# rafaelcgon/2D-GP

Hardware: AMD Instinct MI355X
Metric: posterior grid points/sec (fit+predict), N_train=4096, div-free 2D kernel (higher is better)
Workload: dtype f64 (variance GEMM as exact int8 Ozaki-II); 1 GPU; df kernel, N_train=4096, 256x256 grid per GPU, fit+predict (mean+variance); n_train=4096, grid_per_gpu=256x256, points_total=65536, parallelism=grid-sharded x1, factor local, kstar_ahead=False

## Files before the change

### 2d-gp_amd/csrc/ozaki.hpp

```cpp
#pragma once
#include <climits>
#include <type_traits>
#include "common.hpp"
#include "assemble.hpp"

namespace gp2d {

constexpr int OZ_MAXMOD = 20;
#ifdef GP2D_OZ_P
#define GP2D_OZ_PW GP2D_OZ_P
#define GP2D_OZ_PB GP2D_OZ_P
#endif
#ifndef GP2D_OZ_PW
#define GP2D_OZ_PW 49
#endif
#ifndef GP2D_OZ_PB
#define GP2D_OZ_PB 45
#endif
constexpr int OZ_PW = GP2D_OZ_PW;
constexpr int OZ_PB = GP2D_OZ_PB;
static_assert(OZ_PW <= 50 && OZ_PB <= 50, "ozaki: the one-part residues need |x| < 2^50");
constexpr int OZ_PW_MAX = 60;
constexpr int OZ_PB_MAX = 50;
constexpr int OZ_SPLIT = 26;
constexpr int OZ_HBITS = 33;

struct OzakiConsts {
  int nmod;
  int pw;
  int pb;
  int m[OZ_MAXMOD];
  double c26[OZ_MAXMOD];
  double md[OZ_MAXMOD];
  double inv_m[OZ_MAXMOD];
  double h[OZ_MAXMOD];
  double t[OZ_MAXMOD];
  double M;
  int sB;
  double vlimit;
};

constexpr double OZ_MAGIC52 = 6755399441055744.0;
__device__ __forceinline__ uint32_t residue_low_m(double x, double xm, double m, double inv_m) {
  return (uint32_t)__double_as_longlong(fma(-m, rint(x * inv_m), xm));
}
__device__ __forceinline__ uint32_t pack2_lo(uint32_t a, uint32_t b) { return __builtin_amdgcn_perm(b, a, 0x0c0c0400u); }
__device__ __forceinline__ uint32_t pack22(uint32_t a, uint32_t b) { return __builtin_amdgcn_perm(b, a, 0x05040100u); }

__host__ __device__ __forceinline__ int64_t slab_offset(int64_t row, int64_t k, int64_t K) {
  return (((row >> 8) * (K >> 6) + (k >> 6)) << 14) + ((row & 255) << 6) + (k & 63);
}

__device__ __forceinline__ double block_reduce(double v, double* red, bool is_max) {
  const int tid = threadIdx.x;
  red[tid] = v;
  __syncthreads();
  for (int s = 128; s > 0; s >>= 1) {
    if (tid < s) red[tid] = is_max ? fmax(red[tid], red[tid + s]) : red[tid] + red[tid + s];
    __syncthreads();
  }
  const double r = red[0];
  __syncthreads();
  return r;
}

struct WRows {
  int64_t ldw;
  __device__ __forceinline__ int64_t off(int64_t i) const {
    if (ldw) return i * ldw;
    const int64_t rb = i >> 7;
    return ((rb * (rb + 1)) << 13) + (i & 127) * ((rb + 1) << 7);
  }
  __device__ __forceinline__ int64_t len(int64_t i, int64_t n) const { return ldw ? n : ((i >> 7) + 1) << 7; }
};

__global__ __launch_bounds__(256) void ozaki_w_scale_kernel(const double* __restrict__ W, int64_t n, WRows wr, int pw,
                                                            double* __restrict__ rowscale, double* __restrict__ l1,
                                                            double M, int sB, int final_scale) {
  __shared__ double red[256];
  const int64_t i = blockIdx.x;
  const int tid = threadIdx.x;
  const double* w = W + wr.off(i);
  double mx = 0.0;
  for (int64_t k = tid; k <= i; k += 256) mx = fmax(mx, fabs(w[k]));
  mx = block_reduce(mx, red, true);
  const int e = (mx > 0.0) ? ilogb(mx) : 0;
  const int si = pw - 1 - e;
  double sum = 0.0;
  if (l1 != nullptr) {
    for (int64_t k = tid; k <= i; k += 256) sum += fabs(rint(ldexp(w[k], si)));
    sum = block_reduce(sum, red, false);
  }
  if (tid == 0) {
    rowscale[i] = final_scale ? ldexp(M, -si - sB) : (double)si;
    if (l1 != nullptr) l1[i] = sum;
  }
}

__global__ __launch_bounds__(256) void ozaki_rowscale_final_kernel(double* __restrict__ rowscale, int64_t n, double M,
                                                                   int sB) {
  const int64_t i = (int64_t)blockIdx.x * 256 + threadIdx.x;
  if (i < n) rowscale[i] = ldexp(M, -(int)rowscale[i] - sB);
}

__device__ __forceinline__ int ozaki_row_exp(double rowscale_i, const OzakiConsts& oc) {
  return ilogb(oc.M) - ilogb(rowscale_i) - oc.sB;
}

__device__ __forceinline__ void w_residues4(const double (&x)[4], const OzakiConsts& oc, int l, uint32_t (&r)[4]) {
  const double m = oc.md[l], im = oc.inv_m[l];
  if (oc.pw <= 50) {
#pragma unroll
    for (int u = 0; u < 4; ++u) r[u] = residue_low_m(x[u], x[u] + OZ_MAGIC52, m, im);
  } else {
    const double c = oc.c26[l];
#pragma unroll
    for (int u = 0; u < 4; ++u) {
      const double xh = rint(ldexp(x[u], -OZ_SPLIT));
      const double xl = x[u] - ldexp(xh, OZ_SPLIT);
      const double rh = fma(-m, rint(xh * im), xh), rl = fma(-m, rint(xl * im), xl);
      const double t = fma(rh, c, rl);
      r[u] = residue_low_m(t, t + OZ_MAGIC52, m, im);
    }
  }
}
__device__ __forceinline__ uint32_t pack4_lo(const uint32_t (&r)[4]) {
  return pack22(pack2_lo(r[0], r[1]), pack2_lo(r[2], r[3]));
}
__device__ __forceinline__ uint32_t centred_sum(uint32_t a, uint32_t b, int m) {
  int s = (int)a + (int)b;
  const int half = m >> 1;
  s -= (s > half) ? m : 0;
  s += (s < -half) ? m : 0;
  return (uint32_t)s;
}

__global__ __launch_bounds__(256) void ozaki_w_res_kernel(const double* __restrict__ W, int64_t n, WRows wr,
                                                          OzakiConsts oc, int8_t* __restrict__ wres,
                                                          const double* __restrict__ rowscale, int64_t s_npad) {
  const int64_t bi = blockIdx.y, ks = blockIdx.x;
  if (ks * 64 >= (bi + 1) * 256) return;
  const int64_t hs = s_npad / 64;
  const bool fold = hs > 0 && bi * 256 >= s_npad;
  if (fold && ks >= hs) return;
  const bool right = fold && (ks + hs) * 64 < (bi + 1) * 256;
  const int lane = threadIdx.x & 63, wv = threadIdx.x >> 6;
  const int64_t k0 = ks * 64 + 4 * (lane & 15);
  const int64_t plane = n * n;
  auto scaled4 = [&](int64_t i, int64_t kc, int si, double (&x)[4]) {
    const double* w = W + wr.off(i) + kc;
    d2 p0 = {0.0, 0.0}, p1 = {0.0, 0.0};
    if (kc < wr.len(i, n)) {
      p0 = *reinterpret_cast<const d2*>(w);
      p1 = *reinterpret_cast<const d2*>(w + 2);
    }
    const double v[4] = {p0.x, p0.y, p1.x, p1.y};
#pragma unroll
    for (int u = 0; u < 4; ++u) x[u] = (kc + u <= i) ? rint(ldexp(v[u], si)) : 0.0;
  };
#pragma unroll 1
  for (int it = 0; it < 16; ++it) {
    const int64_t i = bi * 256 + wv * 64 + it * 4 + (lane >> 4);
    const int si = ozaki_row_exp(rowscale[i], oc);
    double x[4];
    scaled4(i, k0, si, x);
    int8_t* dst = wres + slab_offset(i, k0, n);
    if (!fold) {
      for (int l = 0; l < oc.nmod; ++l) {
        uint32_t r[4];
        w_residues4(x, oc, l, r);
        *reinterpret_cast<uint32_t*>(dst + (int64_t)l * plane) = pack4_lo(r);
      }
    } else {
      double xr[4] = {0.0, 0.0, 0.0, 0.0};
      if (right) scaled4(i, s_npad + k0, si, xr);
      int8_t* dst_r = wres + slab_offset(i, s_npad + k0, n);
      int8_t* dst_s = wres + slab_offset(i - s_npad, s_npad + k0, n);
      for (int l = 0; l < oc.nmod; ++l) {
        uint32_t r[4], q[4] = {0u, 0u, 0u, 0u};
        w_residues4(x, oc, l, r);
        *reinterpret_cast<uint32_t*>(dst + (int64_t)l * plane) = pack4_lo(r);
        if (right) {
          w_residues4(xr, oc, l, q);
          *reinterpret_cast<uint32_t*>(dst_r + (int64_t)l * plane) = pack4_lo(q);
        }
#pragma unroll
        for (int u = 0; u < 4; ++u) q[u] = centred_sum(r[u], q[u], oc.m[l]);
        *reinterpret_cast<uint32_t*>(dst_s + (int64_t)l * plane) = pack4_lo(q);
      }
    }
  }
}

#ifndef GP2D_KS_OCC
#define GP2D_KS_OCC 5
#endif
#ifndef GP2D_KS_PPL
#define GP2D_KS_PPL 2
#endif
constexpr int OZ_KS_T = 64;
constexpr int OZ_KS_P = 64;
constexpr int OZ_KS_PPL = GP2D_KS_PPL;
static_assert(OZ_KS_PPL == 2 || OZ_KS_PPL == 4, "2 or 4 training points per lane");

template <int PPL> struct packed_bytes;
template <> struct packed_bytes<2> { typedef uint16_t type; };
template <> struct packed_bytes<4> { typedef uint32_t type; };

enum { KS_PLAIN = 0, KS_DIFF_X = 1, KS_DIFF_R = 2 };
template <bool OFF32, int FORM>
__global__ __launch_bounds__(256, GP2D_KS_OCC) void ozaki_kstar_kernel(
    const double* __restrict__ xtr, int64_t ntr, int64_t npad, const double* __restrict__ xg, int64_t cv,
    int64_t cp, VecParams vp, const double* __restrict__ alpha, OzakiConsts oc, int8_t* __restrict__ bres,
    double* __restrict__ pm, uint8_t* __restrict__ flags) {
  constexpr int PPL = OZ_KS_PPL, LG = 64 / PPL, RPW = 64 / LG, RPI = 4 * RPW;
  typedef typename packed_bytes<PPL>::type pk_t;
  const int lane = threadIdx.x & 63, wv = threadIdx.x >> 6;
  const int kg = lane % LG, r = lane / LG;
  const int64_t t0 = (int64_t)blockIdx.x * OZ_KS_T + PPL * kg;
  const int64_t n = 2 * npad, ncols = 2 * cp;
  double a1[PPL], a2[PPL], x0[PPL], x1[PPL], x2[PPL];
  bool tv[PPL];
#pragma unroll
  for (int u = 0; u < PPL; ++u) {
    const int64_t t = t0 + u;
    tv[u] = t < ntr;
    x0[u] = x1[u] = x2[u] = 0.0;
    if (tv[u]) vec_point(vp, xtr, t, x0[u], x1[u], x2[u]);
    a1[u] = (alpha != nullptr && t < npad) ? alpha[t] : 0.0;
    a2[u] = (alpha != nullptr && t < npad) ? alpha[npad + t] : 0.0;
  }
  const double scale = ldexp(1.0, oc.sB);
  bool nz = false;
#pragma unroll 1
  for (int q = 0; q < OZ_KS_P / RPI; ++q) {
    const int64_t p = (int64_t)blockIdx.y * OZ_KS_P + RPI * q + RPW * wv + r;
    const bool pv = p < cv;
    double g0 = 0.0, g1 = 0.0, g2 = 0.0;
    if (pv) vec_point(vp, xg, p, g0, g1, g2);
    double k11[PPL], k12[PPL], k22[PPL];
    double mu = 0.0, mv = 0.0;
#pragma unroll
    for (int u = 0; u < PPL; ++u) {
      if (pv && tv[u]) {
        vec_block_st(vp, x0[u] - g0, x1[u] - g1, x2[u] - g2, k11[u], k12[u], k22[u]);
      } else {
        k11[u] = k12[u] = k22[u] = 0.0;
      }
      mu += a1[u] * k11[u] + a2[u] * k12[u];
      mv += a1[u] * k12[u] + a2[u] * k22[u];
    }
    if (pm != nullptr) {
#pragma unroll
      for (int o = LG / 2; o > 0; o >>= 1) {
        mu += __shfl_xor(mu, o);
        mv += __shfl_xor(mv, o);
      }
      if (kg == 0 && p < cp) {
        pm[(int64_t)blockIdx.x * ncols + p] = mu;
        pm[(int64_t)blockIdx.x * ncols + cp + p] = mv;
      }
    }
    if (p >= cp || t0 >= npad) continue;
    double xi[3][PPL], xm[3][PPL];
#pragma unroll
    for (int u = 0; u < PPL; ++u) {
      xi[0][u] = rint(k11[u] * scale);
      xi[1][u] = rint(k12[u] * scale);
      xi[2][u] = rint(k22[u] * scale);
      if constexpr (FORM == KS_DIFF_X) {
        xi[0][u] -= xi[1][u];
        xi[2][u] -= xi[1][u];
      }
      if constexpr (FORM == KS_DIFF_R) nz = nz || xi[1][u] != 0.0 || xi[0][u] != xi[1][u] || xi[2][u] != xi[1][u];
      else nz = nz || xi[0][u] != 0.0 || xi[1][u] != 0.0 || xi[2][u] != 0.0;
#pragma unroll
      for (int e = 0; e < 3; ++e) xm[e][u] = xi[e][u] + OZ_MAGIC52;
    }
    const int64_t o_uu = slab_offset(p, t0, n), o_uv = slab_offset(p, npad + t0, n),
                  o_vv = slab_offset(cp + p, npad + t0, n);
    const int64_t pstride = ncols * n;
    for (int l = 0; l < oc.nmod; ++l) {
      const double m = oc.md[l], im = oc.inv_m[l];
      pk_t pk[3];
      uint32_t r[3][PPL];
#pragma unroll
      for (int e = 0; e < 3; ++e)
#pragma unroll
        for (int u = 0; u < PPL; ++u) r[e][u] = residue_low_m(xi[e][u], xm[e][u], m, im);
      if constexpr (FORM == KS_DIFF_R) {
#pragma unroll
        for (int u = 0; u < PPL; ++u) {
          r[0][u] = centred_sum(r[0][u], 0u - r[1][u], oc.m[l]);
          r[2][u] = centred_sum(r[2][u], 0u - r[1][u], oc.m[l]);
        }
      }
#pragma unroll
      for (int e = 0; e < 3; ++e) {
        if constexpr (PPL == 2) pk[e] = (pk_t)pack2_lo(r[e][0], r[e][1]);
        else pk[e] = (pk_t)pack22(pack2_lo(r[e][0], r[e][1]), pack2_lo(r[e][2], r[e][3]));
      }
      int8_t* plane = bres + (int64_t)l * pstride;
      if constexpr (OFF32) {
        const __amdgpu_buffer_rsrc_t rs = __builtin_amdgcn_make_buffer_rsrc(plane, (short)0, (int)pstride, 0x00020000);
        if constexpr (PPL == 2) {
          __builtin_amdgcn_raw_buffer_store_b16(pk[0], rs, (int)o_uu, 0, 0);
          __builtin_amdgcn_raw_buffer_store_b16(pk[1], rs, (int)o_uv, 0, 0);
          __builtin_amdgcn_raw_buffer_store_b16(pk[2], rs, (int)o_vv, 0, 0);
        } else {
          __builtin_amdgcn_raw_buffer_store_b32(pk[0], rs, (int)o_uu, 0, 0);
          __builtin_amdgcn_raw_buffer_store_b32(pk[1], rs, (int)o_uv, 0, 0);
          __builtin_amdgcn_raw_buffer_store_b32(pk[2], rs, (int)o_vv, 0, 0);
        }
      } else {
        *reinterpret_cast<pk_t*>(plane + o_uu) = pk[0];
        *reinterpret_cast<pk_t*>(plane + o_uv) = pk[1];
        *reinterpret_cast<pk_t*>(plane + o_vv) = pk[2];
      }
    }
  }
  if (flags != nullptr) {
    const int any = __syncthreads_or(nz ? 1 : 0);
    if (threadIdx.x == 0) flags[(int64_t)blockIdx.y * gridDim.x + blockIdx.x] = any ? 1 : 0;
  }
}

__global__ __launch_bounds__(64) void ozaki_slab_list_kernel(const uint8_t* __restrict__ flags, int ntb, int nbj,
                                                             int kslabs, int* __restrict__ list,
                                                             int* __restrict__ cnt) {
  const int bj = blockIdx.x, lane = threadIdx.x;
  const int g = bj % (nbj / 2);
  const uint8_t* f = flags + (int64_t)(4 * g) * ntb;
  int* L = list + (int64_t)bj * kslabs;
  int* C = cnt + (int64_t)bj * (kslabs / 4 + 1);
  int c = 0;
  for (int s0 = 0; s0 < kslabs; s0 += 64) {
    const int sl = s0 + lane;
    bool keep = false;
    if (sl < kslabs) {
      const int tb = sl % ntb;
      keep = (f[tb] | f[ntb + tb] | f[2 * ntb + tb] | f[3 * ntb + tb]) != 0;
    }
    const uint64_t bal = __ballot(keep);
    const int below = c + __popcll(bal & ((1ull << lane) - 1ull));
    if (keep) L[below] = sl;
    if (sl < kslabs && (sl & 3) == 0) C[sl >> 2] = below;
    c += __popcll(bal);
  }
  if (lane == 0) C[kslabs >> 2] = c;
}

struct OzModConsts {
  int neg_c;
  int neg_m;
  uint32_t magic;
};
__host__ __device__ inline uint32_t ozaki_acc_bias(int K, int m) {
  return (uint32_t)((((int64_t)K << 14) + m - 1) / m * m);
}
__device__ __forceinline__ OzModConsts ozaki_mod_consts(int m) {
  OzModConsts c;
  c.neg_c = -((1 << 20) - (1 << 20) % m);
  c.neg_m = -m;
  c.magic = (uint32_t)(((1u << 29) + (uint32_t)m - 1) / (uint32_t)m);
  return c;
}
__device__ __forceinline__ uint32_t ozaki_mod_u32(uint32_t v, const OzModConsts& c) {
  int y, r;
  uint32_t q;
  asm("v_mad_i32_i24 %0, %1, %2, %3" : "=v"(y) : "v"(v >> 20), "s"(c.neg_c), "v"(v));
  asm("v_mul_hi_u32_u24 %0, %1, %2" : "=v"(q) : "s"(c.magic), "v"(y << 3));
  asm("v_mad_i32_i24 %0, %1, %2, %3" : "=v"(r) : "v"(q), "s"(c.neg_m), "v"(y));
  return (uint32_t)r;
}

constexpr int IBM = 256, IBN = 256, IBK = 64;
constexpr int I_OP = IBM * IBK;
constexpr int I_STAGE = 2 * I_OP;
constexpr int I_NSTAGE = 4;


typedef int i4v __attribute__((ext_vector_type(4)));
typedef __attribute__((address_space(3))) void* lds_ptr_t;

__device__ __forceinline__ void lds_dma16(__amdgpu_buffer_rsrc_t r, lds_ptr_t dst, int voff, int soff) {
#if defined(__HIP_DEVICE_COMPILE__)
  __builtin_amdgcn_raw_ptr_buffer_load_lds(r, dst, 16, voff, soff, 0, 0);
#endif
}

__device__ __forceinline__ int swz16(int row, int chunk) {
  const int q = (row >> 2) & 3;
  const int g = (0x78 >> (2 * q)) & 3;
  return chunk ^ g;
}

template <int P, int W>
__device__ __forceinline__ void vmwait_barrier(std::integral_constant<int, W>) {
  static_assert(P * W < 64, "vmcnt field");
  asm volatile("s_waitcnt vmcnt(%0)\n\ts_waitcnt lgkmcnt(0)\n\ts_barrier" ::"n"(P * W) : "memory");
}

struct IgemmProd {
  int bi0;
  int a_slab0;
  int a_fold;
  int a_fold_slab0;
  int b_rb0;
  int b_slab0;
  int alias_rb, alias_ks;
  int k_bi0, k_cap;
  int c_col0;
  int add_col0;
  static IgemmProd plain(int K, bool lower) {
    return {0, 0, INT_MAX, 0, 0, 0, INT_MAX, 0, lower ? 0 : -(1 << 20), K, 0, -1};
  }
};
struct IgemmZ {
  int64_t sA, sB, sC;
  int m[OZ_MAXMOD];
};
constexpr int64_t kIgemmZBatchMaxN = 4096;

template <int TBN, int NST>
__global__ __launch_bounds__(TBN * 2, (TBN == 256) ? 1 : 2) void igemm_nt_mod_kernel(
    const int8_t* __restrict__ A, const int8_t* __restrict__ B, uint8_t* C, int64_t ldc, int kslabs_i, int modulus,
    const IgemmProd p, const int* __restrict__ slist, const int* __restrict__ scnt, const IgemmZ zb) {
  if (gridDim.z > 1) {
    A += blockIdx.z * zb.sA;
    B += blockIdx.z * zb.sB;
    C += blockIdx.z * zb.sC;
    modulus = zb.m[blockIdx.z];
  }
  static_assert(TBN == 256 || TBN == 128, "tile width");
  static_assert(NST >= 3 && NST <= 5, "ring depth 3..5 (the tail is written out for these)");
  constexpr int NW = TBN / 32;
  constexpr int WC = TBN / 64;
  constexpr int B_OP = TBN * IBK;
  constexpr int STG = I_OP + B_OP;
  constexpr int AP = IBM / NW / 16;
  constexpr int BPW = TBN / NW / 16;
  constexpr int PPW = AP + BPW;
  __shared__ __attribute__((aligned(16))) int8_t smem[NST * STG];
  const int bj = blockIdx.x;
  const int bi = p.bi0 + (int)(gridDim.y - 1 - blockIdx.y);
  const int i0 = bi * IBM, j0 = bj * TBN;
  const int jb = p.b_rb0 + j0 / IBN, jr = j0 % IBN;
  const int ke = min(p.k_cap, (bi - p.k_bi0 + 1) * IBM);
  const bool afold = bi >= p.a_fold;
  const int arb = afold ? bi - p.a_fold : bi, as0 = afold ? p.a_fold_slab0 : p.a_slab0;
  const int tid = threadIdx.x, lane = tid & 63, wid = __builtin_amdgcn_readfirstlane(tid >> 6);
  const int wr = wid / WC, wc = wid % WC;
  const int l16 = lane & 15, lq = lane >> 4;
  const int64_t kslabs = kslabs_i;
  const int8_t* Ap = A + ((int64_t)arb * kslabs + as0) * I_OP;
  const bool alias = jb >= p.alias_rb;
  const int alias_ks = p.alias_ks;
  const int8_t* Bp = B + ((int64_t)jb * kslabs + p.b_slab0) * I_OP + jr * IBK;
  const int8_t* Bq = B + ((int64_t)(alias ? jb - p.alias_rb : 0) * kslabs + alias_ks) * I_OP + jr * IBK;
  int nsl = ke / IBK;
  const int* sl = nullptr;
  if (slist != nullptr) {
    const int* cn = scnt + (int64_t)jb * (kslabs / 4 + 1) + p.b_slab0 / 4;
    const int c0 = cn[0], c = cn[ke / IBM] - c0;
    if (c == 0 || c >= NST - 1) {
      nsl = c;
      sl = slist + (int64_t)jb * kslabs + c0;
    }
  }

  const int bias = (int)ozaki_acc_bias(p.k_cap, modulus);
  i4v acc[8][4];
#pragma unroll
  for (int mi = 0; mi < 8; ++mi)
#pragma unroll
    for (int ni = 0; ni < 4; ++ni) acc[mi][ni] = i4v{bias, bias, bias, bias};

  const int drow = lane >> 2, dchunk = lane & 3;
  const __amdgpu_buffer_rsrc_t rA =
      __builtin_amdgcn_make_buffer_rsrc((void*)Ap, (short)0, (int)((kslabs - as0) * I_OP), 0x00020000);
  const __amdgpu_buffer_rsrc_t rBp =
      __builtin_amdgcn_make_buffer_rsrc((void*)Bp, (short)0, (int)((kslabs - p.b_slab0) * I_OP), 0x00020000);
  const __amdgpu_buffer_rsrc_t rBq =
      __builtin_amdgcn_make_buffer_rsrc((void*)Bq, (short)0, (int)((kslabs - alias_ks) * I_OP), 0x00020000);
  int voA[AP], voB[BPW];
#pragma unroll
  for (int h = 0; h < AP; ++h) {
    const int row = (wid * AP + h) * 16 + drow;
    voA[h] = row * IBK + 16 * swz16(row, dchunk);
  }
#pragma unroll
  for (int h = 0; h < BPW; ++h) {
    const int row = (wid * BPW + h) * 16 + drow;
    voB[h] = row * IBK + 16 * swz16(jr + row, dchunk);
  }
  auto issue = [&](int ks, int st) {
    int8_t* As = smem + st * STG;
    int8_t* Bs = As + I_OP;
    const int so = ks * I_OP;
#pragma unroll
    for (int h = 0; h < AP; ++h) lds_dma16(rA, (lds_ptr_t)(As + (wid * AP + h) * 16 * IBK), voA[h], so);
    const bool q = alias && ks < alias_ks;
#pragma unroll
    for (int h = 0; h < BPW; ++h) lds_dma16(q ? rBq : rBp, (lds_ptr_t)(Bs + (wid * BPW + h) * 16 * IBK), voB[h], so);
  };

  const uint32_t lds_base = (uint32_t)(size_t)(lds_ptr_t)smem;
  const uint32_t lane_a = (uint32_t)((wr * 128 + l16) * IBK + 16 * swz16(l16, lq));
  const uint32_t lane_b = (uint32_t)(I_OP + (wc * 64 + l16) * IBK + 16 * swz16(jr + l16, lq));
  auto reada = [&](int st, int half, i4v (&a)[4]) {
    const uint32_t ad = lds_base + st * STG + lane_a;
    if (half == 0) {
      asm volatile("ds_read_b128 %0, %1 offset:0" : "=v"(a[0]) : "v"(ad) : "memory");
      asm volatile("ds_read_b128 %0, %1 offset:1024" : "=v"(a[1]) : "v"(ad) : "memory");
      asm volatile("ds_read_b128 %0, %1 offset:2048" : "=v"(a[2]) : "v"(ad) : "memory");
      asm volatile("ds_read_b128 %0, %1 offset:3072" : "=v"(a[3]) : "v"(ad) : "memory");
    } else {
      asm volatile("ds_read_b128 %0, %1 offset:4096" : "=v"(a[0]) : "v"(ad) : "memory");
      asm volatile("ds_read_b128 %0, %1 offset:5120" : "=v"(a[1]) : "v"(ad) : "memory");
      asm volatile("ds_read_b128 %0, %1 offset:6144" : "=v"(a[2]) : "v"(ad) : "memory");
      asm volatile("ds_read_b128 %0, %1 offset:7168" : "=v"(a[3]) : "v"(ad) : "memory");
    }
  };
  auto readb = [&](int st, i4v (&b)[4]) {
    const uint32_t ad = lds_base + st * STG + lane_b;
    asm volatile("ds_read_b128 %0, %1 offset:0" : "=v"(b[0]) : "v"(ad) : "memory");
    asm volatile("ds_read_b128 %0, %1 offset:1024" : "=v"(b[1]) : "v"(ad) : "memory");
    asm volatile("ds_read_b128 %0, %1 offset:2048" : "=v"(b[2]) : "v"(ad) : "memory");
    asm volatile("ds_read_b128 %0, %1 offset:3072" : "=v"(b[3]) : "v"(ad) : "memory");
  };
  auto mfmas = [&](int half, const i4v (&a)[4], const i4v (&b)[4]) {
#pragma unroll
    for (int u = 0; u < 4; ++u)
#pragma unroll
      for (int ni = 0; ni < 4; ++ni)
        acc[4 * half + u][ni] = __builtin_amdgcn_mfma_i32_16x16x64_i8(a[u], b[ni], acc[4 * half + u][ni], 0, 0, 0);
  };
  typedef const __attribute__((address_space(4))) int* const_int_ptr;
  const int b_slab0 = p.b_slab0;
  auto slab = [&](int s) -> int { return sl ? ((const_int_ptr)sl)[min(s, nsl - 1)] - b_slab0 : s; };
  if (nsl > 0) {
#pragma unroll
    for (int q = 0; q < NST - 1; ++q) issue(slab(q), q);
    int knext = slab(NST - 1);
    vmwait_barrier<PPW>(std::integral_constant<int, NST - 2>{});
    i4v bA[4], a0A[4], bB[4], a0B[4], a1[4];
    readb(0, bA);
    reada(0, 0, a0A);
    __builtin_amdgcn_sched_barrier(0);
    constexpr int LAST = -1;
    auto step = [&](auto dma_c, auto w_c, int s, i4v (&b)[4], i4v (&a0)[4], i4v (&bn)[4], i4v (&a0n)[4]) {
      constexpr bool dma = decltype(dma_c)::value;
      constexpr int w = decltype(w_c)::value;
      const int st = s % NST;
      if constexpr (dma) {
        issue(knext, (s + NST - 1) % NST);
        knext = slab(s + NST);
      }
      reada(st, 1, a1);
      asm volatile("s_waitcnt lgkmcnt(4)" ::: "memory");
      __builtin_amdgcn_sched_barrier(0);
      mfmas(0, a0, b);
      __builtin_amdgcn_sched_barrier(0);
      if constexpr (w != LAST) {
        vmwait_barrier<PPW>(w_c);
        const int st1 = (s + 1) % NST;
        readb(st1, bn);
        reada(st1, 0, a0n);
        asm volatile("s_waitcnt lgkmcnt(8)" ::: "memory");
      } else {
        asm volatile("s_waitcnt lgkmcnt(0)" ::: "memory");
      }
      __builtin_amdgcn_sched_barrier(0);
      mfmas(1, a1, b);
      __builtin_amdgcn_sched_barrier(0);
    };
    using T_ = std::true_type;
    using F_ = std::false_type;
    using W_FULL = std::integral_constant<int, NST - 2>;
    const int m = nsl - (NST - 1);
    int s = 0;
    for (; s + 1 < m; s += 2) {
      step(T_{}, W_FULL{}, s, bA, a0A, bB, a0B);
      step(T_{}, W_FULL{}, s + 1, bB, a0B, bA, a0A);
    }
    if (s < m) {
      step(T_{}, W_FULL{}, s, bA, a0A, bB, a0B);
      ++s;
#pragma unroll
      for (int u = 0; u < 4; ++u) {
        bA[u] = bB[u];
        a0A[u] = a0B[u];
      }
    }
    if constexpr (NST == 5) {
      step(F_{}, std::integral_constant<int, 2>{}, s, bA, a0A, bB, a0B);
      step(F_{}, std::integral_constant<int, 1>{}, s + 1, bB, a0B, bA, a0A);
      step(F_{}, std::integral_constant<int, 0>{}, s + 2, bA, a0A, bB, a0B);
      step(F_{}, std::integral_constant<int, LAST>{}, s + 3, bB, a0B, bA, a0A);
    } else if constexpr (NST == 4) {
      step(F_{}, std::integral_constant<int, 1>{}, s, bA, a0A, bB, a0B);
      step(F_{}, std::integral_constant<int, 0>{}, s + 1, bB, a0B, bA, a0A);
      step(F_{}, std::integral_constant<int, LAST>{}, s + 2, bA, a0A, bB, a0B);
    } else {
      step(F_{}, std::integral_constant<int, 0>{}, s, bA, a0A, bB, a0B);
      step(F_{}, std::integral_constant<int, LAST>{}, s + 1, bB, a0B, bA, a0A);
    }
    asm volatile("s_waitcnt lgkmcnt(0)\n\ts_barrier" ::: "memory");
  }
  uint8_t* T = reinterpret_cast<uint8_t*>(smem);
  constexpr int TP = IBM + 16;
  static_assert(TBN * TP <= NST * STG, "epilogue image fits the ring");
  const OzModConsts mc = ozaki_mod_consts(modulus);
  constexpr int NP = (IBM * TBN / 16) / (TBN * 2);
  auto epilogue = [&](auto add_c) {
    constexpr bool add = decltype(add_c)::value;
    if constexpr (add) {
      const uint8_t* Cp = C + (int64_t)(p.add_col0 + j0) * ldc + i0;
      i4v pv[NP];
#pragma unroll
      for (int q = 0; q < NP; ++q) {
        const int id = tid + TBN * 2 * q;
        pv[q] = __builtin_nontemporal_load(reinterpret_cast<const i4v*>(Cp + (int64_t)(id >> 4) * ldc + 16 * (id & 15)));
      }
#pragma unroll
      for (int q = 0; q < NP; ++q) {
        const int id = tid + TBN * 2 * q;
        *reinterpret_cast<i4v*>(T + (id >> 4) * TP + 16 * (id & 15)) = pv[q];
      }
      __syncthreads();
    }
#pragma unroll
    for (int mi = 0; mi < 8; ++mi)
#pragma unroll
      for (int ni = 0; ni < 4; ++ni) {
        const int rloc = wr * 128 + mi * 16 + 4 * lq;
        const int cloc = wc * 64 + ni * 16 + l16;
        uint32_t* t = reinterpret_cast<uint32_t*>(T + cloc * TP + rloc);
        uint32_t prior = 0;
        if constexpr (add) prior = *t;
        uint32_t pk = 0;
#pragma unroll
        for (int u = 0; u < 4; ++u)
          pk |= ozaki_mod_u32((uint32_t)acc[mi][ni][u] + ((prior >> (8 * u)) & 0xffu), mc) << (8 * u);
        *t = pk;
      }
  };
  if (p.add_col0 >= 0) epilogue(std::true_type{});
  else epilogue(std::false_type{});
  __syncthreads();
  uint8_t* Cc = C + (int64_t)(p.c_col0 + j0) * ldc + i0;
#pragma unroll
  for (int q = 0; q < NP; ++q) {
    const int id = tid + TBN * 2 * q;
    const int cloc = id >> 4, ch = id & 15;
    const i4v v = *reinterpret_cast<const i4v*>(T + cloc * TP + 16 * ch);
    __builtin_nontemporal_store(v, reinterpret_cast<i4v*>(Cc + (int64_t)cloc * ldc + 16 * ch));
  }
}

constexpr int OZ_GUARD_RSEG = 256;
__global__ __launch_bounds__(256) void ozaki_guard_colsq_kernel(const double* __restrict__ W, int64_t n, int64_t ldw,
                                                                double* __restrict__ psum, double* __restrict__ pmax) {
  const int64_t c = (int64_t)blockIdx.x * 256 + threadIdx.x, seg = blockIdx.y;
  const int64_t r0 = seg * OZ_GUARD_RSEG, r1 = min<int64_t>(n, r0 + OZ_GUARD_RSEG);
  if (c >= n) return;
  double sq = 0.0, mx = 0.0;
  if (r1 > (int64_t)blockIdx.x * 256) {
#pragma unroll 8
    for (int64_t r = r0; r < r1; ++r) {
      const double w = W[r * ldw + c];
      sq = fma(w, w, sq);
      mx = fmax(mx, fabs(w));
    }
  }
  psum[seg * n + c] = sq;
  pmax[seg * n + c] = mx;
}

__global__ __launch_bounds__(1024) void ozaki_guard_finish_kernel(const double* __restrict__ psum,
                                                                  const double* __restrict__ pmax, int64_t n,
                                                                  int64_t nseg, int64_t ntr, int64_t npad, double delta,
                                                                  double* __restrict__ stats) {
  __shared__ double red[2][16];
  const int tid = threadIdx.x, lane = tid & 63, w = tid >> 6;
  double vmin = INFINITY, wmax = 0.0;
  for (int64_t c = tid; c < n; c += 1024) {
    double sq = 0.0, mx = 0.0;
    for (int64_t g = 0; g < nseg; ++g) {
      sq += psum[g * n + c];
      mx = fmax(mx, pmax[g * n + c]);
    }
    wmax = fmax(wmax, mx);
    const int64_t loc = c < npad ? c : c - npad;
    if (loc < ntr) vmin = fmin(vmin, delta * (1.0 - delta * sq));
  }
  for (int o = 32; o > 0; o >>= 1) {
    vmin = fmin(vmin, __shfl_xor(vmin, o));
    wmax = fmax(wmax, __shfl_xor(wmax, o));
  }
  if (lane == 0) { red[0][w] = vmin; red[1][w] = wmax; }
  __syncthreads();
  if (tid == 0) {
    for (int q = 1; q < 16; ++q) { vmin = fmin(vmin, red[0][q]); wmax = fmax(wmax, red[1][q]); }
    stats[0] = vmin;
    stats[1] = wmax;
  }
}

__global__ __launch_bounds__(1024) void morton_bbox_kernel(const double* __restrict__ P, int64_t n, int dim,
                                                           double* __restrict__ bbox) {
  __shared__ double red[2][3][32];
  const int tid = threadIdx.x, lane = tid & 63, w = tid >> 6;
  double lo[3] = {INFINITY, INFINITY, INFINITY}, hi[3] = {-INFINITY, -INFINITY, -INFINITY};
  for (int64_t i = tid; i < n; i += 1024)
    for (int c = 0; c < dim; ++c) {
      const double v = P[i * dim + c];
      lo[c] = fmin(lo[c], v);
      hi[c] = fmax(hi[c], v);
    }
  for (int c = 0; c < dim; ++c) {
    for (int o = 32; o > 0; o >>= 1) {
      lo[c] = fmin(lo[c], __shfl_xor(lo[c], o));
      hi[c] = fmax(hi[c], __shfl_xor(hi[c], o));
    }
    if (lane == 0) { red[0][c][w] = lo[c]; red[1][c][w] = hi[c]; }
  }
  __syncthreads();
  if (tid < dim) {
    double a = INFINITY, b = -INFINITY;
    for (int q = 0; q < 16; ++q) { a = fmin(a, red[0][tid][q]); b = fmax(b, red[1][tid][q]); }
    bbox[tid] = a;
    bbox[3 + tid] = b;
  }
}

__device__ __forceinline__ uint64_t spread2(uint64_t v) {
  v = (v | (v << 16)) & 0x0000FFFF0000FFFFull;
  v = (v | (v << 8)) & 0x00FF00FF00FF00FFull;
  v = (v | (v << 4)) & 0x0F0F0F0F0F0F0F0Full;
  v = (v | (v << 2)) & 0x3333333333333333ull;
  return (v | (v << 1)) & 0x5555555555555555ull;
}
__device__ __forceinline__ uint64_t spread3(uint64_t v) {
  v &= 0x1FFFFFull;
  v = (v | (v << 32)) & 0x001F00000000FFFFull;
  v = (v | (v << 16)) & 0x001F0000FF0000FFull;
  v = (v | (v << 8)) & 0x100F00F00F00F00Full;
  v = (v | (v << 4)) & 0x10C30C30C30C30C3ull;
  return (v | (v << 2)) & 0x1249249249249249ull;
}

__global__ __launch_bounds__(256) void morton_code_kernel(const double* __restrict__ P, int64_t n, int dim,
                                                          const double* __restrict__ bbox,
                                                          int64_t* __restrict__ code) {
  const int64_t i = (int64_t)blockIdx.x * 256 + threadIdx.x;
  if (i >= n) return;
  uint64_t c = 0;
  for (int k = 0; k < dim; ++k) {
    const double lo = bbox[k], span = fmax(bbox[3 + k] - lo, 1e-300);
    double q = rint((P[i * dim + k] - lo) / span * 2097151.0);
    q = fmin(fmax(q, 0.0), 2097151.0);
    const uint64_t v = (uint64_t)q;
    c |= (dim == 2 ? spread2(v) : spread3(v)) << k;
  }
  code[i] = (int64_t)c;
}

#ifndef GP2D_CRT_RPL
#define GP2D_CRT_RPL 16
#endif
constexpr int OZ_CRT_RPL = GP2D_CRT_RPL;
static_assert(OZ_CRT_RPL == 16 || OZ_CRT_RPL == 8, "CRT rows per lane: 16 or 8");
constexpr int OZ_CRT_ROWS = 64 * OZ_CRT_RPL;
constexpr int OZ_CRT_COLS = 4;
constexpr int OZ_CRT_BCOLS = 4 * OZ_CRT_COLS;

template <int RPL> struct crt_load;
template <> struct crt_load<16> { typedef uint4 type; };
template <> struct crt_load<8> { typedef uint2 type; };

#ifndef GP2D_CRT_OCC
#define GP2D_CRT_OCC 1
#endif
__global__ __launch_bounds__(256, GP2D_CRT_OCC) void ozaki_crt_colsq_kernel(const uint8_t* __restrict__ cres, int64_t n,
                                                              int64_t ncols, OzakiConsts oc,
                                                              const double* __restrict__ rowscale,
                                                              double* __restrict__ P) {
  constexpr int RPL = OZ_CRT_RPL;
  typedef typename crt_load<RPL>::type ld_t;
  const int lane = threadIdx.x & 63;
  const int64_t jw = (int64_t)blockIdx.x * OZ_CRT_BCOLS + (threadIdx.x >> 6) * OZ_CRT_COLS;
  const int64_t seg = blockIdx.y;
  const int64_t i0 = seg * OZ_CRT_ROWS + RPL * lane;
  if (jw >= ncols) return;
  const bool rows_ok = i0 < n;
  double rs[RPL];
#pragma unroll
  for (int c = 0; c < RPL; ++c) rs[c] = rows_ok ? rowscale[i0 + c] : 0.0;
  const int64_t plane = n * ncols;
#pragma unroll 1
  for (int jc = 0; jc < OZ_CRT_COLS; ++jc) {
    const int64_t j = jw + jc;
    if (j >= ncols) break;
    double acc = 0.0;
    if (rows_ok) {
      double H[RPL], T[RPL];
#pragma unroll
      for (int c = 0; c < RPL; ++c) { H[c] = 0.0; T[c] = 0.0; }
      const int nm1 = oc.nmod - 1;
      for (int l0 = 0; l0 < oc.nmod; l0 += 4) {
        ld_t v[4];
#pragma unroll
        for (int u = 0; u < 4; ++u)
          v[u] = *reinterpret_cast<const ld_t*>(cres + (int64_t)min(l0 + u, nm1) * plane + j * n + i0);
#pragma unroll
        for (int u = 0; u < 4; ++u) {
          const uint32_t* w = reinterpret_cast<const uint32_t*>(&v[u]);
          const double h = oc.h[l0 + u], t = oc.t[l0 + u];
#pragma unroll
          for (int c = 0; c < RPL; ++c) {
            const double cl = (double)((w[c >> 2] >> (8 * (c & 3))) & 0xffu);
            H[c] = fma(cl, h, H[c]);
            T[c] = fma(cl, t, T[c]);
          }
        }
      }
#pragma unroll
      for (int c = 0; c < RPL; ++c) {
        const double f = (H[c] - rint(H[c])) + T[c];
        const double vij = f * rs[c];
        acc = fma(vij, vij, acc);
        if (fabs(vij) > oc.vlimit) acc = __builtin_nan("");
      }
    }
#pragma unroll
    for (int o = 32; o > 0; o >>= 1) acc += __shfl_xor(acc, o);
    if (lane == 0) P[seg * ncols + j] = acc;
  }
}

}
```

Baseline: 1.295 million points/s.

## Prefetch accumulate-prior tile into freed ring stages via LDS DMA during GEMM tail

The prior C tile (used when accumulating) is now loaded with buffer-to-LDS DMA into the two ring stages that free up during the pipeline drain, so the load overlaps the last MFMA steps instead of running as a serialized global load and LDS store after the main loop. The epilogue image switches from a padded layout to an XOR-swizzled unpadded layout split into two stage-sized halves. The vmcnt waits in the tail are adjusted to account for the extra outstanding DMAs. The 128-wide tile variant is dropped and launch bounds are fixed to one block per SIMD setting, which narrows configuration flexibility.

```diff
diff --git a/2d-gp_amd/csrc/ozaki.hpp b/2d-gp_amd/csrc/ozaki.hpp
--- a/2d-gp_amd/csrc/ozaki.hpp
+++ b/2d-gp_amd/csrc/ozaki.hpp
@@ -395,10 +395,10 @@
   return chunk ^ g;
 }
 
-template <int P, int W>
+template <int P, int X = 0, int W = 0>
 __device__ __forceinline__ void vmwait_barrier(std::integral_constant<int, W>) {
-  static_assert(P * W < 64, "vmcnt field");
-  asm volatile("s_waitcnt vmcnt(%0)\n\ts_waitcnt lgkmcnt(0)\n\ts_barrier" ::"n"(P * W) : "memory");
+  static_assert(P * W + X < 64, "vmcnt field (6 bits)");
+  asm volatile("s_waitcnt vmcnt(%0)\n\ts_waitcnt lgkmcnt(0)\n\ts_barrier" ::"n"(P * W + X) : "memory");
 }
 
 struct IgemmProd {
@@ -422,8 +422,10 @@
 };
 constexpr int64_t kIgemmZBatchMaxN = 4096;
 
+constexpr int I_EPI_HALF = IBM * 128;
+
 template <int TBN, int NST>
-__global__ __launch_bounds__(TBN * 2, (TBN == 256) ? 1 : 2) void igemm_nt_mod_kernel(
+__global__ __launch_bounds__(TBN * 2, 1) void igemm_nt_mod_kernel(
     const int8_t* __restrict__ A, const int8_t* __restrict__ B, uint8_t* C, int64_t ldc, int kslabs_i, int modulus,
     const IgemmProd p, const int* __restrict__ slist, const int* __restrict__ scnt, const IgemmZ zb) {
   if (gridDim.z > 1) {
@@ -432,7 +434,7 @@
     C += blockIdx.z * zb.sC;
     modulus = zb.m[blockIdx.z];
   }
-  static_assert(TBN == 256 || TBN == 128, "tile width");
+  static_assert(TBN == 256, "tile width");
   static_assert(NST >= 3 && NST <= 5, "ring depth 3..5 (the tail is written out for these)");
   constexpr int NW = TBN / 32;
   constexpr int WC = TBN / 64;
@@ -441,6 +443,7 @@
   constexpr int AP = IBM / NW / 16;
   constexpr int BPW = TBN / NW / 16;
   constexpr int PPW = AP + BPW;
+  static_assert(STG == I_EPI_HALF, "a ring stage holds one half of the epilogue image");
   __shared__ __attribute__((aligned(16))) int8_t smem[NST * STG];
   const int bj = blockIdx.x;
   const int bi = p.bi0 + (int)(gridDim.y - 1 - blockIdx.y);
@@ -539,6 +542,24 @@
   typedef const __attribute__((address_space(4))) int* const_int_ptr;
   const int b_slab0 = p.b_slab0;
   auto slab = [&](int s) -> int { return sl ? ((const_int_ptr)sl)[min(s, nsl - 1)] - b_slab0 : s; };
+
+  int8_t* const img0 = smem + ((nsl + 1) % NST) * STG;
+  int8_t* const img1 = smem + (nsl % NST) * STG;
+  const bool add = p.add_col0 >= 0;
+  constexpr int PRI = (IBM * TBN / 1024) / NW;
+  auto issue_prior = [&](int half) {
+    const int ld = (int)ldc;
+    const __amdgpu_buffer_rsrc_t rP = __builtin_amdgcn_make_buffer_rsrc(
+        (void*)(C + (int64_t)(max(p.add_col0, 0) + j0) * ldc + i0), (short)0, add ? (TBN - 1) * ld + IBM : 0, 0x00020000);
+    const int t3 = wid & 3, hf = wid >> 2, cl = lane >> 4;
+    const int vo = cl * ld + 16 * ((lane & 15) ^ (4 * t3 + cl));
+    int8_t* const dst = (half ? img1 : img0) + t3 * 1024;
+#pragma unroll
+    for (int h = 0; h < PRI / 2; ++h) {
+      const int g = hf + 2 * h;
+      lds_dma16(rP, (lds_ptr_t)(dst + g * 4096), vo, (32 * half + 4 * g + t3) * 4 * ld);
+    }
+  };
   if (nsl > 0) {
 #pragma unroll
     for (int q = 0; q < NST - 1; ++q) issue(slab(q), q);
@@ -549,9 +570,10 @@
     reada(0, 0, a0A);
     __builtin_amdgcn_sched_barrier(0);
     constexpr int LAST = -1;
-    auto step = [&](auto dma_c, auto w_c, int s, i4v (&b)[4], i4v (&a0)[4], i4v (&bn)[4], i4v (&a0n)[4]) {
+    auto step = [&](auto dma_c, auto w_c, auto px_c, int s, i4v (&b)[4], i4v (&a0)[4], i4v (&bn)[4], i4v (&a0n)[4]) {
       constexpr bool dma = decltype(dma_c)::value;
       constexpr int w = decltype(w_c)::value;
+      constexpr int px = decltype(px_c)::value;
       const int st = s % NST;
       if constexpr (dma) {
         issue(knext, (s + NST - 1) % NST);
@@ -563,7 +585,7 @@
       mfmas(0, a0, b);
       __builtin_amdgcn_sched_barrier(0);
       if constexpr (w != LAST) {
-        vmwait_barrier<PPW>(w_c);
+        vmwait_barrier<PPW, px>(w_c);
         const int st1 = (s + 1) % NST;
         readb(st1, bn);
         reada(st1, 0, a0n);
@@ -578,14 +600,15 @@
     using T_ = std::true_type;
     using F_ = std::false_type;
     using W_FULL = std::integral_constant<int, NST - 2>;
+    using X0 = std::integral_constant<int, 0>;
     const int m = nsl - (NST - 1);
     int s = 0;
     for (; s + 1 < m; s += 2) {
-      step(T_{}, W_FULL{}, s, bA, a0A, bB, a0B);
-      step(T_{}, W_FULL{}, s + 1, bB, a0B, bA, a0A);
+      step(T_{}, W_FULL{}, X0{}, s, bA, a0A, bB, a0B);
+      step(T_{}, W_FULL{}, X0{}, s + 1, bB, a0B, bA, a0A);
     }
     if (s < m) {
-      step(T_{}, W_FULL{}, s, bA, a0A, bB, a0B);
+      step(T_{}, W_FULL{}, X0{}, s, bA, a0A, bB, a0B);
       ++s;
 #pragma unroll
       for (int u = 0; u < 4; ++u) {
@@ -593,50 +616,40 @@
         a0A[u] = a0B[u];
       }
     }
+    using XH = std::integral_constant<int, PRI / 2>;
+    using X_ = std::integral_constant<int, PRI>;
+    issue_prior(1);
     if constexpr (NST == 5) {
-      step(F_{}, std::integral_constant<int, 2>{}, s, bA, a0A, bB, a0B);
-      step(F_{}, std::integral_constant<int, 1>{}, s + 1, bB, a0B, bA, a0A);
-      step(F_{}, std::integral_constant<int, 0>{}, s + 2, bA, a0A, bB, a0B);
-      step(F_{}, std::integral_constant<int, LAST>{}, s + 3, bB, a0B, bA, a0A);
+      step(F_{}, std::integral_constant<int, 2>{}, XH{}, s, bA, a0A, bB, a0B);
+      issue_prior(0);
+      step(F_{}, std::integral_constant<int, 1>{}, X_{}, s + 1, bB, a0B, bA, a0A);
+      step(F_{}, std::integral_constant<int, 0>{}, X_{}, s + 2, bA, a0A, bB, a0B);
+      step(F_{}, std::integral_constant<int, LAST>{}, X_{}, s + 3, bB, a0B, bA, a0A);
     } else if constexpr (NST == 4) {
-      step(F_{}, std::integral_constant<int, 1>{}, s, bA, a0A, bB, a0B);
-      step(F_{}, std::integral_constant<int, 0>{}, s + 1, bB, a0B, bA, a0A);
-      step(F_{}, std::integral_constant<int, LAST>{}, s + 2, bA, a0A, bB, a0B);
+      step(F_{}, std::integral_constant<int, 1>{}, XH{}, s, bA, a0A, bB, a0B);
+      issue_prior(0);
+      step(F_{}, std::integral_constant<int, 0>{}, X_{}, s + 1, bB, a0B, bA, a0A);
+      step(F_{}, std::integral_constant<int, LAST>{}, X_{}, s + 2, bA, a0A, bB, a0B);
     } else {
-      step(F_{}, std::integral_constant<int, 0>{}, s, bA, a0A, bB, a0B);
-      step(F_{}, std::integral_constant<int, LAST>{}, s + 1, bB, a0B, bA, a0A);
-    }
-    asm volatile("s_waitcnt lgkmcnt(0)\n\ts_barrier" ::: "memory");
-  }
-  uint8_t* T = reinterpret_cast<uint8_t*>(smem);
-  constexpr int TP = IBM + 16;
-  static_assert(TBN * TP <= NST * STG, "epilogue image fits the ring");
+      step(F_{}, std::integral_constant<int, 0>{}, XH{}, s, bA, a0A, bB, a0B);
+      issue_prior(0);
+      step(F_{}, std::integral_constant<int, LAST>{}, X_{}, s + 1, bB, a0B, bA, a0A);
+    }
+  } else if (add) {
+    issue_prior(1);
+    issue_prior(0);
+  }
+  asm volatile("s_waitcnt vmcnt(0)\n\ts_waitcnt lgkmcnt(0)\n\ts_barrier" ::: "memory");
   const OzModConsts mc = ozaki_mod_consts(modulus);
   constexpr int NP = (IBM * TBN / 16) / (TBN * 2);
   auto epilogue = [&](auto add_c) {
     constexpr bool add = decltype(add_c)::value;
-    if constexpr (add) {
-      const uint8_t* Cp = C + (int64_t)(p.add_col0 + j0) * ldc + i0;
-      i4v pv[NP];
-#pragma unroll
-      for (int q = 0; q < NP; ++q) {
-        const int id = tid + TBN * 2 * q;
-        pv[q] = __builtin_nontemporal_load(reinterpret_cast<const i4v*>(Cp + (int64_t)(id >> 4) * ldc + 16 * (id & 15)));
-      }
-#pragma unroll
-      for (int q = 0; q < NP; ++q) {
-        const int id = tid + TBN * 2 * q;
-        *reinterpret_cast<i4v*>(T + (id >> 4) * TP + 16 * (id & 15)) = pv[q];
-      }
-      __syncthreads();
-    }
+    uint8_t* const Tw = reinterpret_cast<uint8_t*>((wc >> 1) ? img1 : img0) + ((wc & 1) * 64 + l16) * IBM + 4 * lq;
 #pragma unroll
     for (int mi = 0; mi < 8; ++mi)
 #pragma unroll
       for (int ni = 0; ni < 4; ++ni) {
-        const int rloc = wr * 128 + mi * 16 + 4 * lq;
-        const int cloc = wc * 64 + ni * 16 + l16;
-        uint32_t* t = reinterpret_cast<uint32_t*>(T + cloc * TP + rloc);
+        uint32_t* t = reinterpret_cast<uint32_t*>(Tw + ni * 16 * IBM + 16 * ((wr * 8 + mi) ^ l16));
         uint32_t prior = 0;
         if constexpr (add) prior = *t;
         uint32_t pk = 0;
@@ -646,7 +659,7 @@
         *t = pk;
       }
   };
-  if (p.add_col0 >= 0) epilogue(std::true_type{});
+  if (add) epilogue(std::true_type{});
   else epilogue(std::false_type{});
   __syncthreads();
   uint8_t* Cc = C + (int64_t)(p.c_col0 + j0) * ldc + i0;
@@ -654,7 +667,8 @@
   for (int q = 0; q < NP; ++q) {
     const int id = tid + TBN * 2 * q;
     const int cloc = id >> 4, ch = id & 15;
-    const i4v v = *reinterpret_cast<const i4v*>(T + cloc * TP + 16 * ch);
+    const uint8_t* Th = reinterpret_cast<const uint8_t*>(q * 32 >= 128 ? img1 : img0);
+    const i4v v = *reinterpret_cast<const i4v*>(Th + (cloc & 127) * IBM + 16 * (ch ^ (cloc & 15)));
     __builtin_nontemporal_store(v, reinterpret_cast<i4v*>(Cc + (int64_t)cloc * ldc + 16 * ch));
   }
 }
```

Result: slower. 1.277 million points/s (-1.4%).
